# zhihao-lin/instant-ngp-pp

Measured on AMD Instinct MI355X. Metric: train rays/sec, higher is better.
Workload: dtype f32

## Files before the change

instant-ngp-pp_amd/build.py:

```python
import hashlib
import os
import shutil
import subprocess

HERE = os.path.dirname(os.path.abspath(__file__))
CSRC = os.path.join(HERE, "csrc")
LIB = os.path.join(HERE, "libngp_hip.so")
LIB_ID = LIB + ".id"
HEADERS = [os.path.join(CSRC, "common.h"), os.path.join(HERE, "..", "include", "ngp_hip.h")]

SOURCES = [
    ("ray_kernels.hip", ["-ffp-contract=off"]),
    ("composite_kernels.hip", []),
    ("grid_kernels.hip", []),
    ("mlp_kernels.hip", []),
    ("mesh_kernels.hip", ["-ffp-contract=off"]),
]
COMMON = ["--offload-arch=gfx950", "-O3", "-fPIC", "-std=c++17", "-Wall", "-Wno-unused-function"]


def _flags():
    extra = os.environ.get("NGP_EXTRA_DEFS", "").split()
    return COMMON + (["-DNGP_AB_VARIANTS"] if os.environ.get("NGP_AB_VARIANTS") else []) + extra


def _hipcc():
    exe = shutil.which("hipcc") or "/opt/rocm/bin/hipcc"
    if not os.path.exists(exe):
        raise RuntimeError("hipcc not found: cannot build libngp_hip.so")
    return exe


def have_hipcc():
    return bool(shutil.which("hipcc")) or os.path.exists("/opt/rocm/bin/hipcc")


def _digest(paths, extra=()):
    h = hashlib.sha256()
    for p in paths:
        h.update(os.path.basename(p).encode())
        with open(p, "rb") as f:
            h.update(f.read())
    for e in extra:
        h.update(e.encode())
    return h.hexdigest()[:16]


def source_id():
    srcs = [os.path.join(CSRC, s) for s, _ in SOURCES] + [os.path.join(CSRC, "build_id.cpp")]
    extra = _flags() + [f for _, fl in SOURCES for f in fl]
    return _digest(srcs + HEADERS, extra)


def built_id():
    try:
        return open(LIB_ID).read().strip()
    except OSError:
        return None


def build(force=False, verbose=False):
    want = source_id()
# ... 52 lines not shown
```

instant-ngp-pp_amd/csrc/mlp_kernels.hip:

```cpp
#include "common.h"
#include <stdlib.h>

#ifdef NGP_AB_VARIANTS
static inline bool ab_flag(const char* name) { return getenv(name) != nullptr; }
static inline long ab_long(const char* name, long dflt) { const char* e = getenv(name); const long v = e ? atol(e) : 0; return v > 0 ? v : dflt; }
#else
static inline constexpr bool ab_flag(const char*) { return false; }
static inline constexpr long ab_long(const char*, long dflt) { return dflt; }
#endif

namespace {

typedef float f32x16 __attribute__((ext_vector_type(16)));

enum { MODE_FWD = 0, MODE_DGRAD = 1, MODE_WGRAD = 2 };

struct GemmArgs {
    const float* A; int64_t lda;
    const float* B; int64_t ldb;
    float* C; int64_t ldc;
    int64_t M, N, K;
    const float* bias;
    float* z_pre;
    int act;
    int64_t k_chunk;
    int vecA, vecB;
    int accumulate;
    float* bias_grad;
    const float* f2_W2; int64_t f2_ldw2; const float* f2_b2; float* f2_out; int64_t f2_ldo; int f2_nout, f2_act;
    float* f2_dact;
    const float* xf_dz2; int64_t xf_lddz2;
    const float* xf_W2; int64_t xf_ldw2;
    int xf_nout, xf_act;
    float* xf_dW2; int64_t xf_lddw2; float* xf_db2;
#ifdef NGP_AB_VARIANTS
    int exp;
#endif
};

__device__ __forceinline__ float softplus_fast(float v)
{
    const float e = __builtin_amdgcn_exp2f(v * 1.4426950408889634f);
    float l = 0.6931471805599453f * __builtin_amdgcn_logf(1.0f + e);
    asm volatile("" : "+v"(l));
    const float r = v < -15.0f ? e : l;
    return v > 20.0f ? v : r;
}

__device__ __forceinline__ float act_fwd(float v, int act)
{
    switch (act) {
        case NGP_ACT_RELU: return v > 0.0f ? v : 0.0f;
        case NGP_ACT_SIGMOID: return 1.0f / (1.0f + __expf(-v));
// ... 421 lines not shown
            const int64_t n = n0 + (wn * TN + tn) * 32 + li;
            if (n >= p.N) continue;
            const float bv = (MODE == MODE_FWD && p.bias) ? p.bias[n] : 0.0f;
#pragma unroll
            for (int r = 0; r < 16; r++) {
                const int64_t m = m0 + (wm * TM + tm) * 32 + (r & 3) + 8 * (r >> 2) + 4 * lh;
                if (m >= p.M) continue;
                float v = acc[tm][tn][r];
                if (MODE == MODE_FWD) {
                    v += bv;
                    if (p.z_pre) p.z_pre[m * p.N + n] = v;
                    p.C[m * p.ldc + n] = act_fwd(v, p.act);
                } else if (MODE == MODE_DGRAD) {
                    if (p.accumulate) v += p.C[m * p.ldc + n];
                    p.C[m * p.ldc + n] = v;
                } else {
                    atomicAdd(p.C + m * p.ldc + n, v);
                }
            }
        }
}

template <int MODE, int WM, int WN, int TM, int TN>
__global__ void __launch_bounds__(256) __attribute__((amdgpu_waves_per_eu(3))) gemm_kernel(GemmArgs p)
{
    gemm_body<MODE, WM, WN, TM, TN, 0>(p);
}

template <int WM, int WN, int TM, int TN, int F2>
__global__ void __launch_bounds__(256) __attribute__((amdgpu_waves_per_eu(3))) gemm_fwd2_kernel(GemmArgs p)
{
    gemm_body<MODE_FWD, WM, WN, TM, TN, 0, F2>(p);
}

template <int MODE, int WM, int WN, int TM, int TN, int XF>
__global__ void __launch_bounds__(256) __attribute__((amdgpu_waves_per_eu(3))) gemm_xf_kernel(GemmArgs p)
{
    gemm_body<MODE, WM, WN, TM, TN, XF>(p);
}

typedef float f32x4 __attribute__((ext_vector_type(4)));

template <int OFF>
__device__ __forceinline__ void stream_load(f32x4& dst, const float* ptr)
{
    asm volatile("global_load_dwordx4 %0, %1, off offset:%2" : "=v"(dst) : "v"(ptr), "n"(OFF) : "memory");
}
template <int N>
__device__ __forceinline__ void stream_wait(f32x4& v)
{
    asm volatile("s_waitcnt vmcnt(%1)" : "+v"(v) : "n"(N));
}

template <int F2, int KQ, int ACT1, int TN>
__global__ void __launch_bounds__(512) mlp_stream_fwd_kernel(GemmArgs p, int n_tiles)
{
    extern __shared__ float smem[];
    constexpr int K = KQ * 8;
    constexpr int LDW = K + 4;
    constexpr int STREAM_VMCNT = KQ - 1 + 4 * TN - 4;
    constexpr int H = 32 * TN;
    float* Ws = smem;
    float* W2s = Ws + H * LDW;
    float* b1s = W2s + F2 * H;
    float* b2s = b1s + H;
    float* stage = b2s + 8;
    const int nthr = blockDim.x, nw = nthr >> 6;
    for (int idx = threadIdx.x; idx < H * (K / 4); idx += nthr) {
        const int n = idx / (K / 4), k4 = (idx - n * (K / 4)) * 4;
        const float4 q = *reinterpret_cast<const float4*>(p.B + (int64_t)n * p.ldb + k4);
        *reinterpret_cast<float4*>(Ws + n * LDW + k4) = q;
    }
    for (int idx = threadIdx.x; idx < F2 * H; idx += nthr) {
        const int o = idx / H, n = idx - o * H;
        W2s[idx] = o < p.f2_nout ? p.f2_W2[o * p.f2_ldw2 + n] : 0.0f;
    }
    if (threadIdx.x < H) b1s[threadIdx.x] = p.bias ? p.bias[threadIdx.x] : 0.0f;
    if (threadIdx.x < F2) b2s[threadIdx.x] = (p.f2_b2 && threadIdx.x < p.f2_nout) ? p.f2_b2[threadIdx.x] : 0.0f;
    __syncthreads();

    const int lane = threadIdx.x & 63, wave = threadIdx.x >> 6;
    const int li = lane & 31, lh = lane >> 5;
    const int stride = gridDim.x * nw;
    int tile = blockIdx.x * nw + wave;
    if (tile >= n_tiles) return;
    f32x4 a[KQ];
    auto row_ptr = [&](int t) {
        int64_t r = (int64_t)t * 32 + li;
        if (r >= p.M) r = p.M - 1;
        return p.A + r * p.lda + 4 * lh;
    };
    {
        const float* src = row_ptr(tile);
#pragma unroll
        for (int q = 0; q < KQ; q++) a[q] = *reinterpret_cast<const f32x4*>(src + 8 * q);
    }
    const int f2_act = p.f2_act, nout = p.f2_nout;
    for (; tile < n_tiles; tile += stride) {
        const int next = tile + stride;
        const float* nsrc = row_ptr(next < n_tiles ? next : tile);
        f32x16 acc[TN];
#pragma unroll
        for (int tn = 0; tn < TN; tn++) {
            const float bv = b1s[tn * 32 + li];
#pragma unroll
            for (int r = 0; r < 16; r++) acc[tn][r] = bv;
        }
        float4 bcur[TN], bnxt[TN];
#pragma unroll
        for (int tn = 0; tn < TN; tn++) bcur[tn] = *reinterpret_cast<const float4*>(Ws + (tn * 32 + li) * LDW + 4 * lh);
#pragma unroll
        for (int q = 0; q < KQ; q++) {
            stream_wait<STREAM_VMCNT>(a[q]);
            const f32x4 av = a[q];
            if (q + 1 < KQ) {
#pragma unroll
                for (int tn = 0; tn < TN; tn++)
                    bnxt[tn] = *reinterpret_cast<const float4*>(Ws + (tn * 32 + li) * LDW + 8 * (q + 1) + 4 * lh);
            }
#pragma unroll
            for (int j = 0; j < 4; j++) {
#pragma unroll
                for (int tn = 0; tn < TN; tn++) {
                    const float bf[4] = {bcur[tn].x, bcur[tn].y, bcur[tn].z, bcur[tn].w};
                    acc[tn] = __builtin_amdgcn_mfma_f32_32x32x2f32(av[j], bf[j], acc[tn], 0, 0, 0);
                }
            }
            switch (q) {
#define STREAM_CASE(Q) case Q: stream_load<32 * Q>(a[Q < KQ ? Q : 0], nsrc); break;
                STREAM_CASE(0) STREAM_CASE(1) STREAM_CASE(2) STREAM_CASE(3) STREAM_CASE(4) STREAM_CASE(5) STREAM_CASE(6)
                STREAM_CASE(7) STREAM_CASE(8) STREAM_CASE(9) STREAM_CASE(10) STREAM_CASE(11) STREAM_CASE(12) STREAM_CASE(13)
                STREAM_CASE(14) STREAM_CASE(15) STREAM_CASE(16) STREAM_CASE(17) STREAM_CASE(18) STREAM_CASE(19)
#undef STREAM_CASE
            }
            __builtin_amdgcn_sched_group_barrier(0x100, 4, 0);
            __builtin_amdgcn_sched_group_barrier(0x008, 16, 0);
            __builtin_amdgcn_sched_barrier(0);
#pragma unroll
            for (int tn = 0; tn < TN; tn++) bcur[tn] = bnxt[tn];
        }
        const int64_t m0 = (int64_t)tile * 32;
        float* stg = stage + wave * 1024;
        constexpr int OGW = F2 < 4 ? F2 : 4;
        constexpr int OGN = (F2 + OGW - 1) / OGW;
#pragma unroll
        for (int og = 0; og < OGN; og++) {
            float part[OGW][16];
#pragma unroll
            for (int o = 0; o < OGW; o++)
#pragma unroll
                for (int r = 0; r < 16; r++) part[o][r] = 0.0f;
#pragma unroll
            for (int tn = 0; tn < TN; tn++) {
                const int n = tn * 32 + li;
                float w2[OGW];
#pragma unroll
                for (int o = 0; o < OGW; o++) w2[o] = W2s[(og * OGW + o) * H + n];
                if (og == 0) {
#pragma unroll
                    for (int r = 0; r < 16; r++) {
                        const float z = acc[tn][r];
                        acc[tn][r] = ACT1 == NGP_ACT_RELU ? fmaxf(z, 0.0f) : (ACT1 == NGP_ACT_SOFTPLUS ? softplus_fast(z) : z);
                    }
#pragma unroll
                    for (int r = 0; r < 16; r++) stg[((r & 3) + 8 * (r >> 2) + 4 * lh) * 32 + li] = acc[tn][r];
#pragma unroll
                    for (int i = 0; i < 4; i++) {
                        const int f = lane + 64 * i, row = f >> 3, c4 = (f & 7) * 4;
                        const float4 v = *reinterpret_cast<const float4*>(stg + row * 32 + c4);
                        if (m0 + row < p.M) *reinterpret_cast<float4*>(p.C + (m0 + row) * p.ldc + tn * 32 + c4) = v;
                    }
                }
#pragma unroll
                for (int r = 0; r < 16; r++)
#pragma unroll
                    for (int o = 0; o < OGW; o++) part[o][r] = fmaf(acc[tn][r], w2[o], part[o][r]);
            }
#pragma unroll
            for (int o = 0; o < OGW; o++) {
                float* v = part[o];
#pragma unroll
                for (int half = 8; half >= 1; half >>= 1) {
                    const int mask = half * 2;
                    const bool up = (li & mask) != 0;
#pragma unroll
                    for (int j = 0; j < half; j++) {
                        float lo = v[j], hi = v[j + half];
                        if constexpr (OGW == 1) asm volatile("" : "+v"(lo), "+v"(hi));
                        const float keep = up ? hi : lo;
                        const float send = up ? lo : hi;
                        v[j] = keep + __shfl_xor(send, mask, 64);
                    }
                }
                const float tot = v[0] + __shfl_xor(v[0], 1, 64);
                const int rr = ((li >> 4) & 1) * 8 + ((li >> 3) & 1) * 4 + ((li >> 2) & 1) * 2 + ((li >> 1) & 1);
                const int64_t m = m0 + (rr & 3) + 8 * (rr >> 2) + 4 * lh;
                const int oo = og * OGW + o;
                if ((li & 1) == 0 && oo < nout && m < p.M) {
                    const float yv = act_fwd(tot + b2s[oo], f2_act);
                    p.f2_out[m * p.f2_ldo + oo] = yv;
                    if (p.f2_dact) p.f2_dact[m * p.f2_ldo + oo] = act_dout(yv, f2_act);
                }
            }
        }
    }
}

template <int OFF>
__device__ __forceinline__ void stream_load1(float& dst, const float* ptr)
{
    asm volatile("global_load_dword %0, %1, off offset:%2" : "=v"(dst) : "v"(ptr), "n"(OFF) : "memory");
}
template <int N>
__device__ __forceinline__ void stream_wait1(float& v)
{
    asm volatile("s_waitcnt vmcnt(%1)" : "+v"(v) : "n"(N));
}


template <int XF, int ACT1>
__global__ void __launch_bounds__(512) mlp_stream_dgrad_kernel(GemmArgs p, int n_tiles)
{
    extern __shared__ float smem[];
    constexpr int KQ = 16, LDW = 132;
    constexpr int STREAM_VMCNT = KQ - 1 + 12;
    float* Wt = smem;
    float* W2s = Wt + 128 * LDW;
    float* stage = W2s + XF * 128;
    const int nthr = blockDim.x, nw = nthr >> 6;
    for (int idx = threadIdx.x; idx < 128 * 128; idx += nthr) {
        const int n = idx >> 7, j = idx & 127;
        Wt[j * LDW + n] = p.B[(int64_t)n * p.ldb + j];
    }
    for (int idx = threadIdx.x; idx < XF * 128; idx += nthr) {
        const int o = idx >> 7, n = idx & 127;
        W2s[idx] = o < p.xf_nout ? p.xf_W2[o * p.xf_ldw2 + n] : 0.0f;
    }
    __syncthreads();

    const int lane = threadIdx.x & 63, wave = threadIdx.x >> 6;
    const int li = lane & 31, lh = lane >> 5;
    const int stride = gridDim.x * nw;
    int tile = blockIdx.x * nw + wave;
    if (tile >= n_tiles) return;
    f32x4 a[KQ];
    float d2[XF];
    auto row_of = [&](int t) {
        int64_t r = (int64_t)t * 32 + li;
        return r < p.M ? r : p.M - 1;
    };
    {
        const int64_t r = row_of(tile);
        const float* src = p.A + r * p.lda + 4 * lh;
#pragma unroll
        for (int q = 0; q < KQ; q++) a[q] = *reinterpret_cast<const f32x4*>(src + 8 * q);
#pragma unroll
        for (int o = 0; o < XF; o++) d2[o] = o < p.xf_nout ? p.xf_dz2[r * p.xf_lddz2 + o] : 0.0f;
    }
    const int nout = p.xf_nout;
    float* stg = stage + wave * 1024;
    for (; tile < n_tiles; tile += stride) {
        const int next = tile + stride;
        const int64_t nr = row_of(next < n_tiles ? next : tile);
        const float* nsrc = p.A + nr * p.lda + 4 * lh;
        const float* ndz2 = p.xf_dz2 + nr * p.xf_lddz2;
        f32x16 acc[4];
#pragma unroll
        for (int tn = 0; tn < 4; tn++)
#pragma unroll
            for (int r = 0; r < 16; r++) acc[tn][r] = 0.0f;
        float dcur[XF];
#pragma unroll
        for (int o = 0; o < XF; o++) {
            stream_wait1<STREAM_VMCNT>(d2[o]);
            dcur[o] = d2[o];
        }
        float4 bcur[4], bnxt[4];
#pragma unroll
        for (int tn = 0; tn < 4; tn++) bcur[tn] = *reinterpret_cast<const float4*>(Wt + (tn * 32 + li) * LDW + 4 * lh);
#pragma unroll
        for (int q = 0; q < KQ; q++) {
            stream_wait<STREAM_VMCNT>(a[q]);
            const f32x4 hv = a[q];
            if (q + 1 < KQ) {
#pragma unroll
                for (int tn = 0; tn < 4; tn++)
                    bnxt[tn] = *reinterpret_cast<const float4*>(Wt + (tn * 32 + li) * LDW + 8 * (q + 1) + 4 * lh);
            }
            float sv[4] = {0.0f, 0.0f, 0.0f, 0.0f};
#pragma unroll
            for (int o = 0; o < XF; o++) {
                const float4 w = *reinterpret_cast<const float4*>(W2s + o * 128 + 8 * q + 4 * lh);
                sv[0] = fmaf(dcur[o], w.x, sv[0]); sv[1] = fmaf(dcur[o], w.y, sv[1]);
                sv[2] = fmaf(dcur[o], w.z, sv[2]); sv[3] = fmaf(dcur[o], w.w, sv[3]);
            }
            float av[4];
#pragma unroll
            for (int j = 0; j < 4; j++) av[j] = sv[j] * act_grad_fast(hv[j], ACT1);
#pragma unroll
            for (int j = 0; j < 4; j++) {
#pragma unroll
                for (int tn = 0; tn < 4; tn++) {
                    const float bf[4] = {bcur[tn].x, bcur[tn].y, bcur[tn].z, bcur[tn].w};
                    acc[tn] = __builtin_amdgcn_mfma_f32_32x32x2f32(av[j], bf[j], acc[tn], 0, 0, 0);
                }
            }
            switch (q) {
#define STREAM_CASE(Q) case Q: stream_load<32 * Q>(a[Q], nsrc); break;
                STREAM_CASE(0) STREAM_CASE(1) STREAM_CASE(2) STREAM_CASE(3) STREAM_CASE(4) STREAM_CASE(5) STREAM_CASE(6)
                STREAM_CASE(7) STREAM_CASE(8) STREAM_CASE(9) STREAM_CASE(10) STREAM_CASE(11) STREAM_CASE(12) STREAM_CASE(13)
                STREAM_CASE(14) STREAM_CASE(15)
#undef STREAM_CASE
            }
            if (q == 0) {
                if (XF > 0) stream_load1<0>(d2[0], ndz2);
                if (XF > 1) stream_load1<4>(d2[XF > 1 ? 1 : 0], ndz2);
                if (XF > 2) stream_load1<8>(d2[XF > 2 ? 2 : 0], ndz2);
                if (XF > 3) stream_load1<12>(d2[XF > 3 ? 3 : 0], ndz2);
            }
            __builtin_amdgcn_sched_barrier(0);
#pragma unroll
            for (int tn = 0; tn < 4; tn++) bcur[tn] = bnxt[tn];
        }
        const int64_t m0 = (int64_t)tile * 32;
#pragma unroll
        for (int tn = 0; tn < 4; tn++) {
#pragma unroll
            for (int r = 0; r < 16; r++) stg[((r & 3) + 8 * (r >> 2) + 4 * lh) * 32 + li] = acc[tn][r];
#pragma unroll
            for (int i = 0; i < 4; i++) {
                const int f = lane + 64 * i, row = f >> 3, c4 = (f & 7) * 4;
                const float4 v = *reinterpret_cast<const float4*>(stg + row * 32 + c4);
                if (m0 + row < p.M) *reinterpret_cast<float4*>(p.C + (m0 + row) * p.ldc + tn * 32 + c4) = v;
            }
        }
    }
    (void)nout;
}

template <int XF, int ACT1, int TN, bool W2G>
__global__ void __launch_bounds__(512) mlp_stream_wgrad_kernel(GemmArgs p, int64_t chunk)
{
    extern __shared__ float lds[];
#ifndef NGP_WGRAD_D
#define NGP_WGRAD_D 8
#endif
    constexpr int D = NGP_WGRAD_D;
    const int lane = threadIdx.x & 63, wave = __builtin_amdgcn_readfirstlane((int)((threadIdx.x >> 6) & 3)),
              grp = __builtin_amdgcn_readfirstlane((int)(threadIdx.x >> 8));
    const int li = lane & 31, lh = lane >> 5;
    const bool two = blockDim.x == 512;
    const int64_t half = two ? chunk / 2 : chunk;
    const int64_t cbeg = (int64_t)blockIdx.x * chunk;
    const int64_t cend = cbeg + chunk < p.K ? cbeg + chunk : p.K;
    const int64_t kbeg = cbeg + grp * half < cend ? cbeg + grp * half : cend;
    const int64_t kend = grp == 0 ? (cbeg + half < cend ? cbeg + half : cend) : cend;
    const int h = wave * 32 + li;
    const int N = (int)p.N;
    float w2[XF];
#pragma unroll
    for (int o = 0; o < XF; o++) w2[o] = p.xf_W2[o * p.xf_ldw2 + h];
    f32x16 acc[TN];
#pragma unroll
    for (int tn = 0; tn < TN; tn++)
#pragma unroll
        for (int r = 0; r < 16; r++) acc[tn][r] = 0.0f;
    float gw[XF], gb2[XF], gb1 = 0.0f;
#pragma unroll
    for (int o = 0; o < XF; o++) { gw[o] = 0.0f; gb2[o] = 0.0f; }

    static_assert(D == 8, "a turn of the staging tile is 16 samples = 8 steps");
    float* stg = lds + (two ? (threadIdx.x >> 6) * 1152 : wave * 2048);
    float* sH = stg;
    float* sX5 = stg + 512;
    float* sD = stg + 1024;
// ... 739 lines not shown
        hipLaunchKernelGGL((gemm_kernel<MODE_FWD, 4, 1, 1, 1>), grid, dim3(256), 0, st, p);
    }
    return ngp_check_launch();
}

static int mlp2_fwd_impl(const float* x, int64_t ldx, const float* W1, int64_t ldw1, const float* b1, int act1,
                         const float* W2, int64_t ldw2, const float* b2, int act2, int64_t n, int n_in, int H, int n_out,
                         float* hidden, int64_t ldh, float* out, int64_t ldo, float* dact, void* stream);

int ngp_mlp2_fwd(const float* x, int64_t ldx, const float* W1, int64_t ldw1, const float* b1, int act1,
                 const float* W2, int64_t ldw2, const float* b2, int act2, int64_t n, int n_in, int H, int n_out,
                 float* hidden, int64_t ldh, float* out, int64_t ldo, void* stream)
{
    return mlp2_fwd_impl(x, ldx, W1, ldw1, b1, act1, W2, ldw2, b2, act2, n, n_in, H, n_out, hidden, ldh, out, ldo, nullptr,
                         stream);
}

int ngp_mlp2_fwd_dact(const float* x, int64_t ldx, const float* W1, int64_t ldw1, const float* b1, int act1,
                      const float* W2, int64_t ldw2, const float* b2, int act2, int64_t n, int n_in, int H, int n_out,
                      float* hidden, int64_t ldh, float* out, int64_t ldo, float* dact_out, void* stream)
{
    if (n > 0 && !dact_out) return NGP_EINVAL;
    return mlp2_fwd_impl(x, ldx, W1, ldw1, b1, act1, W2, ldw2, b2, act2, n, n_in, H, n_out, hidden, ldh, out, ldo, dact_out,
                         stream);
}

static int mlp2_fwd_impl(const float* x, int64_t ldx, const float* W1, int64_t ldw1, const float* b1, int act1,
                         const float* W2, int64_t ldw2, const float* b2, int act2, int64_t n, int n_in, int H, int n_out,
                         float* hidden, int64_t ldh, float* out, int64_t ldo, float* dact, void* stream)
{
    if (n < 0 || n_in < 1 || H < 1 || H > 128 || n_out < 1 || n_out > 8 || ldx < n_in || ldw1 < n_in || ldh < H ||
        ldw2 < H || ldo < n_out)
        return NGP_EINVAL;
    if (n == 0) return NGP_OK;
    if (!x || !W1 || !W2 || !hidden || !out) return NGP_EINVAL;
    hipStream_t st = (hipStream_t)stream;
    GemmArgs p{};
    p.A = x; p.lda = ldx; p.B = W1; p.ldb = ldw1; p.C = hidden; p.ldc = ldh;
    p.M = n; p.N = H; p.K = n_in; p.bias = b1; p.act = act1;
    p.vecA = aligned16(x) && (ldx % 4 == 0); p.vecB = aligned16(W1) && (ldw1 % 4 == 0);
    p.f2_W2 = W2; p.f2_ldw2 = ldw2; p.f2_b2 = b2; p.f2_out = out; p.f2_ldo = ldo; p.f2_nout = n_out; p.f2_act = act2;
    p.f2_dact = dact;
    dim3 grid(ngp_blocks(n, 128), 1);
    static const bool stream_ok = !ab_flag("NGP_MLP_NO_STREAM");
    const bool wide_ok = H == 128 && (n_in == 128 || n_in == 144 || n_in == 160);
    static const bool stream_heads = ab_flag("NGP_MLP_STREAM_HEADS");
    const bool head_ok = stream_heads && H == 32 && n_in == 128;
    if (stream_ok && (wide_ok || head_ok) && p.vecA && p.vecB &&
        (act1 == NGP_ACT_RELU || act1 == NGP_ACT_SOFTPLUS) && aligned16(hidden) && ldh % 4 == 0 &&
        n <= (int64_t)32 * 0x7fffff00) {
        const int n_tiles = (int)((n + 31) / 32);
        const int f2 = n_out == 1 ? 1 : (n_out <= 4 ? 4 : 8);
        static const int nw = (int)ab_long("NGP_MLP_NW_FWD", ab_long("NGP_MLP_NW", 8));
        const size_t lds = (size_t)(H * (n_in + 4) + f2 * H + H + 8 + nw * 1024) * sizeof(float);
        static int n_cu = 0;
        if (!n_cu) {
            int dev = 0;
            hipDeviceProp_t prop;
            if (hipGetDevice(&dev) != hipSuccess || hipGetDeviceProperties(&prop, dev) != hipSuccess) return NGP_ELAUNCH;
            n_cu = prop.multiProcessorCount > 0 ? prop.multiProcessorCount : 256;
        }
        static const int wg_rounds_f = (int)ab_long("NGP_MLP_WG_ROUNDS_FWD", ab_long("NGP_MLP_WG_ROUNDS", 1));
        const int max_blocks = n_cu * (H == 128 ? 1 : 2) * wg_rounds_f;
        const int blocks = (n_tiles + nw - 1) / nw < max_blocks ? (n_tiles + nw - 1) / nw : max_blocks;
#define LAUNCH_STREAM(F2V, KQV, ACTV, TNV)                                                                              \
    do {                                                                                                                \
        static bool attr_set = false;                                                                                   \
        if (!attr_set) {                                                                                                \
            if (hipFuncSetAttribute(reinterpret_cast<const void*>(&mlp_stream_fwd_kernel<F2V, KQV, ACTV, TNV>),         \
                                    hipFuncAttributeMaxDynamicSharedMemorySize, 128 * 1024) != hipSuccess)              \
                return NGP_ELAUNCH;                                                                                     \
            attr_set = true;                                                                                            \
        }                                                                                                               \
        hipLaunchKernelGGL((mlp_stream_fwd_kernel<F2V, KQV, ACTV, TNV>), dim3(blocks), dim3(64 * nw), lds, st, p, n_tiles); \
    } while (0)
#define LAUNCH_STREAM_A(F2V, KQV, TNV)                                                                                  \
    do {                                                                                                                \
        if (act1 == NGP_ACT_RELU) LAUNCH_STREAM(F2V, KQV, NGP_ACT_RELU, TNV);                                           \
        else LAUNCH_STREAM(F2V, KQV, NGP_ACT_SOFTPLUS, TNV);                                                            \
    } while (0)
#define LAUNCH_STREAM_K(F2V)                                                                                            \
    do {                                                                                                                \
        if (H == 32) LAUNCH_STREAM_A(F2V, 16, 1);                                                                       \
        else if (n_in == 128) LAUNCH_STREAM_A(F2V, 16, 4);                                                              \
        else if (n_in == 144) LAUNCH_STREAM_A(F2V, 18, 4);                                                              \
        else LAUNCH_STREAM_A(F2V, 20, 4);                                                                               \
    } while (0)
        if (f2 == 1) LAUNCH_STREAM_K(1);
        else if (f2 == 4) LAUNCH_STREAM_K(4);
        else LAUNCH_STREAM_K(8);
#undef LAUNCH_STREAM_K
#undef LAUNCH_STREAM_A
#undef LAUNCH_STREAM
        return ngp_check_launch();
    }
    if (H > 32) {
        if (n_out == 1) hipLaunchKernelGGL((gemm_fwd2_kernel<2, 2, 2, 2, 1>), grid, dim3(256), 0, st, p);
        else if (n_out <= 4) hipLaunchKernelGGL((gemm_fwd2_kernel<2, 2, 2, 2, 4>), grid, dim3(256), 0, st, p);
        else hipLaunchKernelGGL((gemm_fwd2_kernel<2, 2, 2, 2, 8>), grid, dim3(256), 0, st, p);
    } else {
        if (n_out == 1) hipLaunchKernelGGL((gemm_fwd2_kernel<4, 1, 1, 1, 1>), grid, dim3(256), 0, st, p);
        else if (n_out <= 4) hipLaunchKernelGGL((gemm_fwd2_kernel<4, 1, 1, 1, 4>), grid, dim3(256), 0, st, p);
        else hipLaunchKernelGGL((gemm_fwd2_kernel<4, 1, 1, 1, 8>), grid, dim3(256), 0, st, p);
    }
    return ngp_check_launch();
}

int ngp_linear_bwd_input(const float* dz, int64_t lddz, const float* W, int64_t ldw, int64_t n, int n_in, int n_out,
                         float* dx, int64_t lddx, int accumulate, void* stream)
{
    if (n < 0 || n_in < 1 || n_out < 1 || lddz < n_out || ldw < n_in || lddx < n_in) return NGP_EINVAL;
    if (n == 0) return NGP_OK;
    if (!dz || !W || !dx) return NGP_EINVAL;
    hipStream_t st = (hipStream_t)stream;
    if (n_out <= 4) {
        hipLaunchKernelGGL(skinny_dgrad_kernel, dim3(ngp_blocks(n * n_in, 256)), dim3(256), 0, st, dz, lddz, W, ldw, n,
                           n_in, n_out, dx, lddx, accumulate);
        return ngp_check_launch();
    }
    GemmArgs p{};
    p.A = dz; p.lda = lddz; p.B = W; p.ldb = ldw; p.C = dx; p.ldc = lddx;
    p.M = n; p.N = n_in; p.K = n_out; p.act = 0; p.k_chunk = 0; p.accumulate = accumulate;
    p.vecA = aligned16(dz) && (lddz % 4 == 0); p.vecB = aligned16(W) && (ldw % 4 == 0);
    launch_dgrad<0>(p, st);
    return ngp_check_launch();
}

int ngp_linear_bwd_weight(const float* dz, int64_t lddz, const float* x, int64_t ldx, int64_t n, int n_in, int n_out,
                          float* dW, int64_t ldw, float* db, void* stream)
{
    if (n < 0 || n_in < 1 || n_out < 1 || lddz < n_out || ldx < n_in || ldw < n_in) return NGP_EINVAL;
    if (n == 0) return NGP_OK;
    if (!dz || !x || !dW) return NGP_EINVAL;
    hipStream_t st = (hipStream_t)stream;
    if (n_out <= 4) {
        if (n_in > 256) return NGP_EINVAL;
        int cw = 1;
        while (cw < n_in) cw <<= 1;
        const int rpb = 512;
        hipLaunchKernelGGL(skinny_wgrad_kernel, dim3(ngp_blocks(n, rpb)), dim3(256), 0, st, dz, lddz, x, ldx, n, n_in,
                           n_out, cw, rpb, dW, ldw, db);
        return ngp_check_launch();
    }
    GemmArgs p{};
    p.A = dz; p.lda = lddz; p.B = x; p.ldb = ldx; p.C = dW; p.ldc = ldw;
    p.M = n_out; p.N = n_in; p.K = n; p.act = 0; p.bias_grad = db;
// ... 34 lines not shown
{
    if (n < 0 || n_out < 1 || n_out > 16 || !(H == 32 || H == 64 || H == 128)) return NGP_EINVAL;
    if ((dW2 && (lddw2 < H || n_out > 4)) || (db2 && !dW2)) return NGP_EINVAL;
    if (n == 0) return NGP_OK;
    if (!out || !W2 || !hidden || !dz1) return NGP_EINVAL;
    if (((uintptr_t)hidden & 15) || ((uintptr_t)dz1 & 15) || (ldh % 4) || (lddz1 % 4)) return NGP_EINVAL;
    const int rows_per_block = 256 / (H / 4);
    int64_t blocks = (n + rows_per_block - 1) / rows_per_block;
    if (blocks > 8192) blocks = 8192;
    if (dW2 && blocks > 1024) blocks = 1024;
    hipStream_t st = (hipStream_t)stream;
    if (dW2)
        hipLaunchKernelGGL((mlp_hidden_bwd_kernel<4, true>), dim3((unsigned)blocks), dim3(256), 0, st, dOut, lddo, out,
                           ldo, act2, W2, ldw2, hidden, ldh, act1, n, H, n_out, dz2, lddz2, dz1, lddz1, dW2, lddw2, db2);
    else if (n_out <= 4)
        hipLaunchKernelGGL((mlp_hidden_bwd_kernel<4, false>), dim3((unsigned)blocks), dim3(256), 0, st, dOut, lddo, out,
                           ldo, act2, W2, ldw2, hidden, ldh, act1, n, H, n_out, dz2, lddz2, dz1, lddz1, nullptr, 0,
                           nullptr);
    else
        hipLaunchKernelGGL((mlp_hidden_bwd_kernel<16, false>), dim3((unsigned)blocks), dim3(256), 0, st, dOut, lddo, out,
                           ldo, act2, W2, ldw2, hidden, ldh, act1, n, H, n_out, dz2, lddz2, dz1, lddz1, nullptr, 0,
                           nullptr);
    return ngp_check_launch();
}

int ngp_mlp_bwd_input(const float* dz2, int64_t lddz2, const float* W2, int64_t ldw2, const float* hidden,
                      int64_t ldh, int act1, const float* W1, int64_t ldw1, int64_t n, int n_in, int H, int n_out,
                      float* dx, int64_t lddx, int accumulate, void* stream)
{
    if (n < 0 || n_in < 1 || n_out < 1 || n_out > XF_OMAX || H < 8 || ldw1 < n_in || lddx < n_in) return NGP_EINVAL;
    if (n == 0) return NGP_OK;
    if (!xf_args_ok(dz2, lddz2, W2, ldw2, hidden, ldh, H, n_out) || !W1 || !dx) return NGP_EINVAL;
    GemmArgs p{};
    p.A = hidden; p.lda = ldh; p.B = W1; p.ldb = ldw1; p.C = dx; p.ldc = lddx;
    p.M = n; p.N = n_in; p.K = H; p.accumulate = accumulate;
    p.vecA = aligned16(hidden) && (ldh % 4 == 0); p.vecB = aligned16(W1) && (ldw1 % 4 == 0);
    p.xf_dz2 = dz2; p.xf_lddz2 = lddz2; p.xf_W2 = W2; p.xf_ldw2 = ldw2; p.xf_nout = n_out; p.xf_act = act1;
    static const bool stream_ok = !ab_flag("NGP_MLP_NO_STREAM");
    if (stream_ok && H == 128 && n_in == 128 && !accumulate && p.vecA && aligned16(dx) && lddx % 4 == 0 &&
        (act1 == NGP_ACT_RELU || act1 == NGP_ACT_SOFTPLUS) && n <= (int64_t)32 * 0x7fffff00) {
        hipStream_t st = (hipStream_t)stream;
        const int n_tiles = (int)((n + 31) / 32);
        static int n_cu = 0;
        if (!n_cu) {
            int dev = 0;
            hipDeviceProp_t prop;
            if (hipGetDevice(&dev) != hipSuccess || hipGetDeviceProperties(&prop, dev) != hipSuccess) return NGP_ELAUNCH;
            n_cu = prop.multiProcessorCount > 0 ? prop.multiProcessorCount : 256;
        }
        static const int nw = (int)ab_long("NGP_MLP_NW_DGRAD", ab_long("NGP_MLP_NW", 8));
        static const int wg_rounds_d = (int)ab_long("NGP_MLP_WG_ROUNDS_DGRAD", ab_long("NGP_MLP_WG_ROUNDS", 1));
        const int cap_d = n_cu * wg_rounds_d;
        const int blocks = (n_tiles + nw - 1) / nw < cap_d ? (n_tiles + nw - 1) / nw : cap_d;
#define LAUNCH_SD(XFV, ACTV)                                                                                            \
    do {                                                                                                                \
        static bool attr_set = false;                                                                                   \
        const size_t lds = (size_t)(128 * 132 + XFV * 128 + nw * 1024) * sizeof(float);                                 \
        if (!attr_set) {                                                                                                \
            if (hipFuncSetAttribute(reinterpret_cast<const void*>(&mlp_stream_dgrad_kernel<XFV, ACTV>),                 \
                                    hipFuncAttributeMaxDynamicSharedMemorySize, 128 * 1024) != hipSuccess)              \
                return NGP_ELAUNCH;                                                                                     \
            attr_set = true;                                                                                            \
        }                                                                                                               \
        hipLaunchKernelGGL((mlp_stream_dgrad_kernel<XFV, ACTV>), dim3(blocks), dim3(64 * nw), lds, st, p, n_tiles);    \
    } while (0)
#define LAUNCH_SD_A(XFV)                                                                                                \
    do {                                                                                                                \
        if (act1 == NGP_ACT_RELU) LAUNCH_SD(XFV, NGP_ACT_RELU);                                                         \
        else LAUNCH_SD(XFV, NGP_ACT_SOFTPLUS);                                                                          \
    } while (0)
        if (n_out == 1) LAUNCH_SD_A(1);
        else if (n_out == 2) LAUNCH_SD_A(2);
        else if (n_out == 3) LAUNCH_SD_A(3);
        else LAUNCH_SD_A(4);
#undef LAUNCH_SD_A
#undef LAUNCH_SD
        return ngp_check_launch();
    }
    if (n_out == 1) launch_dgrad<1>(p, (hipStream_t)stream);
    else if (n_out <= 3) launch_dgrad<3>(p, (hipStream_t)stream);
    else launch_dgrad<XF_OMAX>(p, (hipStream_t)stream);
    return ngp_check_launch();
}

int ngp_mlp_bwd_weight(const float* dz2, int64_t lddz2, const float* W2, int64_t ldw2, const float* hidden,
                       int64_t ldh, int act1, const float* x, int64_t ldx, int64_t n, int n_in, int H, int n_out,
                       float* dW1, int64_t ldw, float* db1, float* dW2, int64_t lddw2, float* db2, void* stream)
{
    if (n < 0 || n_in < 1 || n_out < 1 || n_out > XF_OMAX || H < 8 || ldx < n_in || ldw < n_in ||
        (dW2 && lddw2 < H) || (db2 && !dW2))
        return NGP_EINVAL;
    if (n == 0) return NGP_OK;
    if (!xf_args_ok(dz2, lddz2, W2, ldw2, hidden, ldh, H, n_out) || !x || !dW1) return NGP_EINVAL;
    GemmArgs p{};
    p.A = hidden; p.lda = ldh; p.B = x; p.ldb = ldx; p.C = dW1; p.ldc = ldw;
    p.M = H; p.N = n_in; p.K = n; p.bias_grad = db1;
    p.vecA = aligned16(hidden) && (ldh % 4 == 0); p.vecB = aligned16(x) && (ldx % 4 == 0);
    p.xf_dz2 = dz2; p.xf_lddz2 = lddz2; p.xf_W2 = W2; p.xf_ldw2 = ldw2; p.xf_nout = n_out; p.xf_act = act1;
    p.xf_dW2 = dW2; p.xf_lddw2 = lddw2; p.xf_db2 = db2;
#ifdef NGP_AB_VARIANTS
    static const int wgrad_exp = getenv("NGP_WGRAD_EXP") ? atoi(getenv("NGP_WGRAD_EXP")) : 0;
    p.exp = wgrad_exp;
#endif
    static const bool stream_ok = !ab_flag("NGP_MLP_NO_STREAM") && !ab_flag("NGP_MLP_NO_STREAM_WGRAD");
    if (stream_ok && H == 128 && (n_in == 128 || n_in == 144 || n_in == 160) && p.vecA && p.vecB &&
        (act1 == NGP_ACT_RELU || act1 == NGP_ACT_SOFTPLUS)) {
        hipStream_t st = (hipStream_t)stream;
        static int n_cu = 0;
        if (!n_cu) {
            int dev = 0;
            hipDeviceProp_t prop;
            if (hipGetDevice(&dev) != hipSuccess || hipGetDeviceProperties(&prop, dev) != hipSuccess) return NGP_ELAUNCH;
            n_cu = prop.multiProcessorCount > 0 ? prop.multiProcessorCount : 256;
        }
        static const int wpc_env = (int)ab_long("NGP_WGRAD_WPC", 1);
        const int wpc = wpc_env == 9 ? 0 : wpc_env;
        const int threads = (n_in == 128 && !wpc) ? 512 : 256;
        int64_t blocks = (int64_t)n_cu * (wpc ? wpc : (threads == 512 ? 1 : 2));
        int64_t chunk = ((n + blocks - 1) / blocks + 31) / 32 * 32;
        if (chunk < 128) chunk = 128;
        {
            int64_t ldmax = ldx > ldh ? ldx : ldh;
            if (lddz2 > ldmax) ldmax = lddz2;
            const int64_t cap = (((int64_t)1 << 31) / (4 * ldmax) - 64) / 32 * 32;
            if (cap < 128) return NGP_EINVAL;
            if (chunk > cap) chunk = cap;
        }
        blocks = (n + chunk - 1) / chunk;
#define LAUNCH_SW2(XFV, ACTV, TNV, W2GV)                                                                                \
// ... 166 lines not shown
```

Before: 2.087 million.

## Emulate f32 MLP GEMMs with 3-way bf16 split on bf16 MFMA

Replaces the f32 MFMA (32x32x2) inner loops in the streaming MLP forward and dgrad kernels with a bf16x3 split emulation. Each operand is split into three bf16 planes and multiplied with six 32x32x16 bf16 MFMAs per 16-deep slice. Weights are pre-split into packed bf16 planes in LDS, which changes the LDS layout and raises the shared-memory limit to 160KB. The aim is higher matrix-core throughput than native f32 MFMA, at the cost of extra VALU split work, more LDS space, and slightly different rounding.

```diff
diff --git a/instant-ngp-pp_amd/build.py b/instant-ngp-pp_amd/build.py
--- a/instant-ngp-pp_amd/build.py
+++ b/instant-ngp-pp_amd/build.py
@@ -7,7 +7,7 @@
 CSRC = os.path.join(HERE, "csrc")
 LIB = os.path.join(HERE, "libngp_hip.so")
 LIB_ID = LIB + ".id"
-HEADERS = [os.path.join(CSRC, "common.h"), os.path.join(HERE, "..", "include", "ngp_hip.h")]
+HEADERS = [os.path.join(CSRC, "common.h"), os.path.join(CSRC, "bf16_split.h"), os.path.join(HERE, "..", "include", "ngp_hip.h")]
 
 SOURCES = [
     ("ray_kernels.hip", ["-ffp-contract=off"]),
diff --git a/instant-ngp-pp_amd/csrc/bf16_split.h b/instant-ngp-pp_amd/csrc/bf16_split.h
--- /dev/null
+++ b/instant-ngp-pp_amd/csrc/bf16_split.h
@@ -0,0 +1,34 @@
+#pragma once
+#include <stdint.h>
+
+#if defined(__HIPCC__)
+#define NGP_SPLIT_FN __host__ __device__ __forceinline__
+#else
+#define NGP_SPLIT_FN static inline
+#endif
+
+NGP_SPLIT_FN uint32_t ngp_f32_bits(float x) { return __builtin_bit_cast(uint32_t, x); }
+NGP_SPLIT_FN float ngp_bits_f32(uint32_t u) { return __builtin_bit_cast(float, u); }
+NGP_SPLIT_FN float ngp_split_sub(float x, float y)
+{
+#if defined(__HIP_DEVICE_COMPILE__)
+    float r;
+    asm("v_sub_f32 %0, %1, %2" : "=v"(r) : "v"(x), "v"(y));
+    return r;
+#else
+    return x - y;
+#endif
+}
+
+NGP_SPLIT_FN void ngp_split_bf16_pair(float x, float y, uint32_t& p1, uint32_t& p2, uint32_t& p3)
+{
+    const uint32_t ux = ngp_f32_bits(x), uy = ngp_f32_bits(y);
+    const uint32_t hx = ux & 0xffff0000u, hy = uy & 0xffff0000u;
+    p1 = (ux >> 16) | hy;
+    const float rx = ngp_split_sub(x, ngp_bits_f32(hx)), ry = ngp_split_sub(y, ngp_bits_f32(hy));
+    const uint32_t urx = ngp_f32_bits(rx), ury = ngp_f32_bits(ry);
+    const uint32_t mx = urx & 0xffff0000u, my = ury & 0xffff0000u;
+    p2 = (urx >> 16) | my;
+    const float sx = ngp_split_sub(rx, ngp_bits_f32(mx)), sy = ngp_split_sub(ry, ngp_bits_f32(my));
+    p3 = (ngp_f32_bits(sx) >> 16) | (ngp_f32_bits(sy) & 0xffff0000u);
+}
diff --git a/instant-ngp-pp_amd/csrc/mlp_kernels.hip b/instant-ngp-pp_amd/csrc/mlp_kernels.hip
--- a/instant-ngp-pp_amd/csrc/mlp_kernels.hip
+++ b/instant-ngp-pp_amd/csrc/mlp_kernels.hip
@@ -1,4 +1,5 @@
 #include "common.h"
+#include "bf16_split.h"
 #include <stdlib.h>
 
 #ifdef NGP_AB_VARIANTS
@@ -526,16 +527,76 @@
     asm volatile("s_waitcnt vmcnt(%1)" : "+v"(v) : "n"(N));
 }
 
-template <int F2, int KQ, int ACT1, int TN>
+typedef __bf16 bf16x8 __attribute__((ext_vector_type(8)));
+typedef uint32_t u32x4 __attribute__((ext_vector_type(4)));
+
+__device__ __forceinline__ void split_frag(const float (&lo)[4], const float (&hi)[4], u32x4 (&s)[3])
+{
+    uint32_t w[3][4];
+    ngp_split_bf16_pair(lo[0], lo[1], w[0][0], w[1][0], w[2][0]);
+    ngp_split_bf16_pair(lo[2], lo[3], w[0][1], w[1][1], w[2][1]);
+    ngp_split_bf16_pair(hi[0], hi[1], w[0][2], w[1][2], w[2][2]);
+    ngp_split_bf16_pair(hi[2], hi[3], w[0][3], w[1][3], w[2][3]);
+#pragma unroll
+    for (int pl = 0; pl < 3; pl++) s[pl] = u32x4{w[pl][0], w[pl][1], w[pl][2], w[pl][3]};
+}
+
+__device__ __forceinline__ void mfma_split6(const u32x4 (&a)[3], const u32x4 (&b)[3], f32x16& acc)
+{
+    constexpr int ai[6] = {2, 1, 0, 1, 0, 0}, bi[6] = {0, 1, 2, 0, 1, 0};
+#pragma unroll
+    for (int t = 0; t < 6; t++)
+        acc = __builtin_amdgcn_mfma_f32_32x32x16_bf16(__builtin_bit_cast(bf16x8, a[ai[t]]), __builtin_bit_cast(bf16x8, b[bi[t]]),
+                                                      acc, 0, 0, 0);
+}
+
+template <int TN, typename LoadB>
+__device__ __forceinline__ void split_slice(const u32x4 (&a)[3], u32x4 (&b0)[3], f32x16 (&acc)[TN], int c, bool more,
+                                            LoadB load_b)
+{
+    u32x4 b[TN][3];
+#pragma unroll
+    for (int pl = 0; pl < 3; pl++) b[0][pl] = b0[pl];
+#pragma unroll
+    for (int tn = 1; tn < TN; tn++) load_b(b[tn], tn, c);
+#pragma unroll
+    for (int tn = 0; tn < TN; tn++) {
+        mfma_split6(a, b[tn], acc[tn]);
+        if (tn == 0 && more) load_b(b0, 0, c + 1);
+    }
+}
+
+__host__ __device__ constexpr int split_ldwb(int K) { return K == 160 ? K : K + 8; }
+__device__ __forceinline__ int split_quad_pos(int Q) { return (Q & ~3) | ((Q & 1) << 1) | ((Q >> 1) & 1); }
+__device__ __forceinline__ void split_store_quad(uint16_t* planes, int plane_stride, int off, float x, float y, float z,
+                                                 float w)
+{
+    uint32_t a1, a2, a3, b1, b2, b3;
+    ngp_split_bf16_pair(x, y, a1, a2, a3);
+    ngp_split_bf16_pair(z, w, b1, b2, b3);
+    *reinterpret_cast<uint2*>(planes + off) = make_uint2(a1, b1);
+    *reinterpret_cast<uint2*>(planes + plane_stride + off) = make_uint2(a2, b2);
+    *reinterpret_cast<uint2*>(planes + 2 * plane_stride + off) = make_uint2(a3, b3);
+}
+
+__host__ __device__ constexpr int stream_fwd_w_floats(bool split, int H, int K)
+{
+    return split ? 3 * H * split_ldwb(K) / 2 : H * (K + 4);
+}
+
+template <int F2, int KQ, int ACT1, int TN, bool SPLIT>
 __global__ void __launch_bounds__(512) mlp_stream_fwd_kernel(GemmArgs p, int n_tiles)
 {
     extern __shared__ float smem[];
     constexpr int K = KQ * 8;
     constexpr int LDW = K + 4;
+    constexpr int LDWB = split_ldwb(K);
     constexpr int STREAM_VMCNT = KQ - 1 + 4 * TN - 4;
     constexpr int H = 32 * TN;
+    static_assert(!SPLIT || KQ % 2 == 0, "split slices are 16 deep");
     float* Ws = smem;
-    float* W2s = Ws + H * LDW;
+    uint16_t* Wb = reinterpret_cast<uint16_t*>(smem);
+    float* W2s = Ws + stream_fwd_w_floats(SPLIT, H, K);
     float* b1s = W2s + F2 * H;
     float* b2s = b1s + H;
     float* stage = b2s + 8;
@@ -543,7 +604,8 @@
     for (int idx = threadIdx.x; idx < H * (K / 4); idx += nthr) {
         const int n = idx / (K / 4), k4 = (idx - n * (K / 4)) * 4;
         const float4 q = *reinterpret_cast<const float4*>(p.B + (int64_t)n * p.ldb + k4);
-        *reinterpret_cast<float4*>(Ws + n * LDW + k4) = q;
+        if constexpr (SPLIT) split_store_quad(Wb, H * LDWB, n * LDWB + 4 * split_quad_pos(k4 >> 2), q.x, q.y, q.z, q.w);
+        else *reinterpret_cast<float4*>(Ws + n * LDW + k4) = q;
     }
     for (int idx = threadIdx.x; idx < F2 * H; idx += nthr) {
         const int o = idx / H, n = idx - o * H;
@@ -580,26 +642,7 @@
 #pragma unroll
             for (int r = 0; r < 16; r++) acc[tn][r] = bv;
         }
-        float4 bcur[TN], bnxt[TN];
-#pragma unroll
-        for (int tn = 0; tn < TN; tn++) bcur[tn] = *reinterpret_cast<const float4*>(Ws + (tn * 32 + li) * LDW + 4 * lh);
-#pragma unroll
-        for (int q = 0; q < KQ; q++) {
-            stream_wait<STREAM_VMCNT>(a[q]);
-            const f32x4 av = a[q];
-            if (q + 1 < KQ) {
-#pragma unroll
-                for (int tn = 0; tn < TN; tn++)
-                    bnxt[tn] = *reinterpret_cast<const float4*>(Ws + (tn * 32 + li) * LDW + 8 * (q + 1) + 4 * lh);
-            }
-#pragma unroll
-            for (int j = 0; j < 4; j++) {
-#pragma unroll
-                for (int tn = 0; tn < TN; tn++) {
-                    const float bf[4] = {bcur[tn].x, bcur[tn].y, bcur[tn].z, bcur[tn].w};
-                    acc[tn] = __builtin_amdgcn_mfma_f32_32x32x2f32(av[j], bf[j], acc[tn], 0, 0, 0);
-                }
-            }
+        auto issue = [&](int q) {
             switch (q) {
 #define STREAM_CASE(Q) case Q: stream_load<32 * Q>(a[Q < KQ ? Q : 0], nsrc); break;
                 STREAM_CASE(0) STREAM_CASE(1) STREAM_CASE(2) STREAM_CASE(3) STREAM_CASE(4) STREAM_CASE(5) STREAM_CASE(6)
@@ -607,11 +650,56 @@
                 STREAM_CASE(14) STREAM_CASE(15) STREAM_CASE(16) STREAM_CASE(17) STREAM_CASE(18) STREAM_CASE(19)
 #undef STREAM_CASE
             }
+        };
+        if constexpr (SPLIT) {
+            auto load_b = [&](u32x4 (&b)[3], int tn, int c) {
+#pragma unroll
+                for (int pl = 0; pl < 3; pl++)
+                    b[pl] = *reinterpret_cast<const u32x4*>(Wb + pl * H * LDWB + (tn * 32 + li) * LDWB + 16 * c + 8 * lh);
+            };
+            u32x4 b0[3];
+            load_b(b0, 0, 0);
+#pragma unroll
+            for (int c = 0; c < KQ / 2; c++) {
+                stream_wait<STREAM_VMCNT>(a[2 * c]);
+                stream_wait<STREAM_VMCNT - 1>(a[2 * c + 1]);
+                const float lo[4] = {a[2 * c][0], a[2 * c][1], a[2 * c][2], a[2 * c][3]};
+                const float hi[4] = {a[2 * c + 1][0], a[2 * c + 1][1], a[2 * c + 1][2], a[2 * c + 1][3]};
+                u32x4 as[3];
+                split_frag(lo, hi, as);
+                split_slice<TN>(as, b0, acc, c, c + 1 < KQ / 2, load_b);
+                issue(2 * c);
+                issue(2 * c + 1);
+                __builtin_amdgcn_sched_barrier(0);
+            }
+        } else {
+        float4 bcur[TN], bnxt[TN];
+#pragma unroll
+        for (int tn = 0; tn < TN; tn++) bcur[tn] = *reinterpret_cast<const float4*>(Ws + (tn * 32 + li) * LDW + 4 * lh);
+#pragma unroll
+        for (int q = 0; q < KQ; q++) {
+            stream_wait<STREAM_VMCNT>(a[q]);
+            const f32x4 av = a[q];
+            if (q + 1 < KQ) {
+#pragma unroll
+                for (int tn = 0; tn < TN; tn++)
+                    bnxt[tn] = *reinterpret_cast<const float4*>(Ws + (tn * 32 + li) * LDW + 8 * (q + 1) + 4 * lh);
+            }
+#pragma unroll
+            for (int j = 0; j < 4; j++) {
+#pragma unroll
+                for (int tn = 0; tn < TN; tn++) {
+                    const float bf[4] = {bcur[tn].x, bcur[tn].y, bcur[tn].z, bcur[tn].w};
+                    acc[tn] = __builtin_amdgcn_mfma_f32_32x32x2f32(av[j], bf[j], acc[tn], 0, 0, 0);
+                }
+            }
+            issue(q);
             __builtin_amdgcn_sched_group_barrier(0x100, 4, 0);
             __builtin_amdgcn_sched_group_barrier(0x008, 16, 0);
             __builtin_amdgcn_sched_barrier(0);
 #pragma unroll
             for (int tn = 0; tn < TN; tn++) bcur[tn] = bnxt[tn];
+        }
         }
         const int64_t m0 = (int64_t)tile * 32;
         float* stg = stage + wave * 1024;
@@ -692,19 +780,31 @@
 }
 
 
-template <int XF, int ACT1>
+__host__ __device__ constexpr int stream_dgrad_w_floats(bool split) { return split ? 3 * 128 * split_ldwb(128) / 2 : 128 * 132; }
+
+template <int XF, int ACT1, bool SPLIT>
 __global__ void __launch_bounds__(512) mlp_stream_dgrad_kernel(GemmArgs p, int n_tiles)
 {
     extern __shared__ float smem[];
-    constexpr int KQ = 16, LDW = 132;
+    constexpr int KQ = 16, LDW = 132, LDWB = split_ldwb(128);
     constexpr int STREAM_VMCNT = KQ - 1 + 12;
     float* Wt = smem;
-    float* W2s = Wt + 128 * LDW;
+    uint16_t* Wb = reinterpret_cast<uint16_t*>(smem);
+    float* W2s = Wt + stream_dgrad_w_floats(SPLIT);
     float* stage = W2s + XF * 128;
     const int nthr = blockDim.x, nw = nthr >> 6;
-    for (int idx = threadIdx.x; idx < 128 * 128; idx += nthr) {
-        const int n = idx >> 7, j = idx & 127;
-        Wt[j * LDW + n] = p.B[(int64_t)n * p.ldb + j];
+    if constexpr (SPLIT) {
+        for (int idx = threadIdx.x; idx < 128 * 32; idx += nthr) {
+            const int j = idx & 127, Q = idx >> 7;
+            const float* src = p.B + (int64_t)(4 * Q) * p.ldb + j;
+            split_store_quad(Wb, 128 * LDWB, j * LDWB + 4 * split_quad_pos(Q), src[0], src[p.ldb], src[2 * p.ldb],
+                             src[3 * p.ldb]);
+        }
+    } else {
+        for (int idx = threadIdx.x; idx < 128 * 128; idx += nthr) {
+            const int n = idx >> 7, j = idx & 127;
+            Wt[j * LDW + n] = p.B[(int64_t)n * p.ldb + j];
+        }
     }
     for (int idx = threadIdx.x; idx < XF * 128; idx += nthr) {
         const int o = idx >> 7, n = idx & 127;
@@ -749,36 +849,7 @@
             stream_wait1<STREAM_VMCNT>(d2[o]);
             dcur[o] = d2[o];
         }
-        float4 bcur[4], bnxt[4];
-#pragma unroll
-        for (int tn = 0; tn < 4; tn++) bcur[tn] = *reinterpret_cast<const float4*>(Wt + (tn * 32 + li) * LDW + 4 * lh);
-#pragma unroll
-        for (int q = 0; q < KQ; q++) {
-            stream_wait<STREAM_VMCNT>(a[q]);
-            const f32x4 hv = a[q];
-            if (q + 1 < KQ) {
-#pragma unroll
-                for (int tn = 0; tn < 4; tn++)
-                    bnxt[tn] = *reinterpret_cast<const float4*>(Wt + (tn * 32 + li) * LDW + 8 * (q + 1) + 4 * lh);
-            }
-            float sv[4] = {0.0f, 0.0f, 0.0f, 0.0f};
-#pragma unroll
-            for (int o = 0; o < XF; o++) {
-                const float4 w = *reinterpret_cast<const float4*>(W2s + o * 128 + 8 * q + 4 * lh);
-                sv[0] = fmaf(dcur[o], w.x, sv[0]); sv[1] = fmaf(dcur[o], w.y, sv[1]);
-                sv[2] = fmaf(dcur[o], w.z, sv[2]); sv[3] = fmaf(dcur[o], w.w, sv[3]);
-            }
-            float av[4];
-#pragma unroll
-            for (int j = 0; j < 4; j++) av[j] = sv[j] * act_grad_fast(hv[j], ACT1);
-#pragma unroll
-            for (int j = 0; j < 4; j++) {
-#pragma unroll
-                for (int tn = 0; tn < 4; tn++) {
-                    const float bf[4] = {bcur[tn].x, bcur[tn].y, bcur[tn].z, bcur[tn].w};
-                    acc[tn] = __builtin_amdgcn_mfma_f32_32x32x2f32(av[j], bf[j], acc[tn], 0, 0, 0);
-                }
-            }
+        auto issue = [&](int q) {
             switch (q) {
 #define STREAM_CASE(Q) case Q: stream_load<32 * Q>(a[Q], nsrc); break;
                 STREAM_CASE(0) STREAM_CASE(1) STREAM_CASE(2) STREAM_CASE(3) STREAM_CASE(4) STREAM_CASE(5) STREAM_CASE(6)
@@ -792,9 +863,73 @@
                 if (XF > 2) stream_load1<8>(d2[XF > 2 ? 2 : 0], ndz2);
                 if (XF > 3) stream_load1<12>(d2[XF > 3 ? 3 : 0], ndz2);
             }
+        };
+        auto fma1 = [](float a, float b, float c) {
+            float r;
+            asm("v_fma_f32 %0, %1, %2, %3" : "=v"(r) : "v"(a), "v"(b), "v"(c));
+            return r;
+        };
+        auto form = [&](int q, const f32x4& hv, float (&av)[4]) {
+            float sv[4] = {0.0f, 0.0f, 0.0f, 0.0f};
+#pragma unroll
+            for (int o = 0; o < XF; o++) {
+                const float4 w = *reinterpret_cast<const float4*>(W2s + o * 128 + 8 * q + 4 * lh);
+                sv[0] = fma1(dcur[o], w.x, sv[0]); sv[1] = fma1(dcur[o], w.y, sv[1]);
+                sv[2] = fma1(dcur[o], w.z, sv[2]); sv[3] = fma1(dcur[o], w.w, sv[3]);
+            }
+#pragma unroll
+            for (int j = 0; j < 4; j++) av[j] = sv[j] * act_grad_fast(hv[j], ACT1);
+        };
+        if constexpr (SPLIT) {
+            auto load_b = [&](u32x4 (&b)[3], int tn, int c) {
+#pragma unroll
+                for (int pl = 0; pl < 3; pl++)
+                    b[pl] = *reinterpret_cast<const u32x4*>(Wb + pl * 128 * LDWB + (tn * 32 + li) * LDWB + 16 * c + 8 * lh);
+            };
+            u32x4 b0[3];
+            load_b(b0, 0, 0);
+#pragma unroll
+            for (int c = 0; c < KQ / 2; c++) {
+                stream_wait<STREAM_VMCNT>(a[2 * c]);
+                stream_wait<STREAM_VMCNT - 1>(a[2 * c + 1]);
+                float lo[4], hi[4];
+                form(2 * c, a[2 * c], lo);
+                form(2 * c + 1, a[2 * c + 1], hi);
+                u32x4 as[3];
+                split_frag(lo, hi, as);
+                split_slice<4>(as, b0, acc, c, c + 1 < KQ / 2, load_b);
+                issue(2 * c);
+                issue(2 * c + 1);
+                __builtin_amdgcn_sched_barrier(0);
+            }
+        } else {
+        float4 bcur[4], bnxt[4];
+#pragma unroll
+        for (int tn = 0; tn < 4; tn++) bcur[tn] = *reinterpret_cast<const float4*>(Wt + (tn * 32 + li) * LDW + 4 * lh);
+#pragma unroll
+        for (int q = 0; q < KQ; q++) {
+            stream_wait<STREAM_VMCNT>(a[q]);
+            const f32x4 hv = a[q];
+            if (q + 1 < KQ) {
+#pragma unroll
+                for (int tn = 0; tn < 4; tn++)
+                    bnxt[tn] = *reinterpret_cast<const float4*>(Wt + (tn * 32 + li) * LDW + 8 * (q + 1) + 4 * lh);
+            }
+            float av[4];
+            form(q, hv, av);
+#pragma unroll
+            for (int j = 0; j < 4; j++) {
+#pragma unroll
+                for (int tn = 0; tn < 4; tn++) {
+                    const float bf[4] = {bcur[tn].x, bcur[tn].y, bcur[tn].z, bcur[tn].w};
+                    acc[tn] = __builtin_amdgcn_mfma_f32_32x32x2f32(av[j], bf[j], acc[tn], 0, 0, 0);
+                }
+            }
+            issue(q);
             __builtin_amdgcn_sched_barrier(0);
 #pragma unroll
             for (int tn = 0; tn < 4; tn++) bcur[tn] = bnxt[tn];
+        }
         }
         const int64_t m0 = (int64_t)tile * 32;
 #pragma unroll
@@ -1640,7 +1775,8 @@
         const int n_tiles = (int)((n + 31) / 32);
         const int f2 = n_out == 1 ? 1 : (n_out <= 4 ? 4 : 8);
         static const int nw = (int)ab_long("NGP_MLP_NW_FWD", ab_long("NGP_MLP_NW", 8));
-        const size_t lds = (size_t)(H * (n_in + 4) + f2 * H + H + 8 + nw * 1024) * sizeof(float);
+        const bool split = !ab_flag("NGP_MLP_F32");
+        const size_t lds = (size_t)(stream_fwd_w_floats(split, H, n_in) + f2 * H + H + 8 + nw * 1024) * sizeof(float);
         static int n_cu = 0;
         if (!n_cu) {
             int dev = 0;
@@ -1651,17 +1787,27 @@
         static const int wg_rounds_f = (int)ab_long("NGP_MLP_WG_ROUNDS_FWD", ab_long("NGP_MLP_WG_ROUNDS", 1));
         const int max_blocks = n_cu * (H == 128 ? 1 : 2) * wg_rounds_f;
         const int blocks = (n_tiles + nw - 1) / nw < max_blocks ? (n_tiles + nw - 1) / nw : max_blocks;
-#define LAUNCH_STREAM(F2V, KQV, ACTV, TNV)                                                                              \
+#define LAUNCH_STREAM_S(F2V, KQV, ACTV, TNV, SPV)                                                                        \
     do {                                                                                                                \
         static bool attr_set = false;                                                                                   \
         if (!attr_set) {                                                                                                \
-            if (hipFuncSetAttribute(reinterpret_cast<const void*>(&mlp_stream_fwd_kernel<F2V, KQV, ACTV, TNV>),         \
-                                    hipFuncAttributeMaxDynamicSharedMemorySize, 128 * 1024) != hipSuccess)              \
+            if (hipFuncSetAttribute(reinterpret_cast<const void*>(&mlp_stream_fwd_kernel<F2V, KQV, ACTV, TNV, SPV>),    \
+                                    hipFuncAttributeMaxDynamicSharedMemorySize, 160 * 1024) != hipSuccess)              \
                 return NGP_ELAUNCH;                                                                                     \
             attr_set = true;                                                                                            \
         }                                                                                                               \
-        hipLaunchKernelGGL((mlp_stream_fwd_kernel<F2V, KQV, ACTV, TNV>), dim3(blocks), dim3(64 * nw), lds, st, p, n_tiles); \
+        hipLaunchKernelGGL((mlp_stream_fwd_kernel<F2V, KQV, ACTV, TNV, SPV>), dim3(blocks), dim3(64 * nw), lds, st, p,     \
+                           n_tiles);                                                                                    \
     } while (0)
+#ifdef NGP_AB_VARIANTS
+#define LAUNCH_STREAM(F2V, KQV, ACTV, TNV)                                                                              \
+    do {                                                                                                                \
+        if (split) LAUNCH_STREAM_S(F2V, KQV, ACTV, TNV, true);                                                          \
+        else LAUNCH_STREAM_S(F2V, KQV, ACTV, TNV, false);                                                               \
+    } while (0)
+#else
+#define LAUNCH_STREAM(F2V, KQV, ACTV, TNV) LAUNCH_STREAM_S(F2V, KQV, ACTV, TNV, true)
+#endif
 #define LAUNCH_STREAM_A(F2V, KQV, TNV)                                                                                  \
     do {                                                                                                                \
         if (act1 == NGP_ACT_RELU) LAUNCH_STREAM(F2V, KQV, NGP_ACT_RELU, TNV);                                           \
@@ -1680,6 +1826,8 @@
 #undef LAUNCH_STREAM_K
 #undef LAUNCH_STREAM_A
 #undef LAUNCH_STREAM
+#undef LAUNCH_STREAM_S
+        (void)split;
         return ngp_check_launch();
     }
     if (H > 32) {
@@ -1820,18 +1968,28 @@
         static const int wg_rounds_d = (int)ab_long("NGP_MLP_WG_ROUNDS_DGRAD", ab_long("NGP_MLP_WG_ROUNDS", 1));
         const int cap_d = n_cu * wg_rounds_d;
         const int blocks = (n_tiles + nw - 1) / nw < cap_d ? (n_tiles + nw - 1) / nw : cap_d;
-#define LAUNCH_SD(XFV, ACTV)                                                                                            \
+        const bool split = !ab_flag("NGP_MLP_F32");
+#define LAUNCH_SD_S(XFV, ACTV, SPV)                                                                                     \
     do {                                                                                                                \
         static bool attr_set = false;                                                                                   \
-        const size_t lds = (size_t)(128 * 132 + XFV * 128 + nw * 1024) * sizeof(float);                                 \
+        const size_t lds = (size_t)(stream_dgrad_w_floats(SPV) + XFV * 128 + nw * 1024) * sizeof(float);                \
         if (!attr_set) {                                                                                                \
-            if (hipFuncSetAttribute(reinterpret_cast<const void*>(&mlp_stream_dgrad_kernel<XFV, ACTV>),                 \
-                                    hipFuncAttributeMaxDynamicSharedMemorySize, 128 * 1024) != hipSuccess)              \
+            if (hipFuncSetAttribute(reinterpret_cast<const void*>(&mlp_stream_dgrad_kernel<XFV, ACTV, SPV>),            \
+                                    hipFuncAttributeMaxDynamicSharedMemorySize, 160 * 1024) != hipSuccess)              \
                 return NGP_ELAUNCH;                                                                                     \
             attr_set = true;                                                                                            \
         }                                                                                                               \
-        hipLaunchKernelGGL((mlp_stream_dgrad_kernel<XFV, ACTV>), dim3(blocks), dim3(64 * nw), lds, st, p, n_tiles);    \
+        hipLaunchKernelGGL((mlp_stream_dgrad_kernel<XFV, ACTV, SPV>), dim3(blocks), dim3(64 * nw), lds, st, p, n_tiles); \
     } while (0)
+#ifdef NGP_AB_VARIANTS
+#define LAUNCH_SD(XFV, ACTV)                                                                                            \
+    do {                                                                                                                \
+        if (split) LAUNCH_SD_S(XFV, ACTV, true);                                                                        \
+        else LAUNCH_SD_S(XFV, ACTV, false);                                                                             \
+    } while (0)
+#else
+#define LAUNCH_SD(XFV, ACTV) LAUNCH_SD_S(XFV, ACTV, true)
+#endif
 #define LAUNCH_SD_A(XFV)                                                                                                \
     do {                                                                                                                \
         if (act1 == NGP_ACT_RELU) LAUNCH_SD(XFV, NGP_ACT_RELU);                                                         \
@@ -1843,6 +2001,8 @@
         else LAUNCH_SD_A(4);
 #undef LAUNCH_SD_A
 #undef LAUNCH_SD
+#undef LAUNCH_SD_S
+        (void)split;
         return ngp_check_launch();
     }
     if (n_out == 1) launch_dgrad<1>(p, (hipStream_t)stream);
```

New measurement: 2.137 million, median of 6. 1.02x the previous value.
